# imaginateit/csm-train-pytorch

Measured on AMD Instinct MI355X. Metric: train tokens/sec (text+audio) CSM-1B bf16 seq2048, higher is better.
Workload: dtype bf16

## Files before the change

csm-train-pytorch_amd/csm/hip/__init__.py:

```python
import ctypes as C
import os

_HERE = os.path.dirname(os.path.abspath(__file__))
LIB_PATH = os.environ.get("CSM_HIP_LIB") or os.path.join(_HERE, "libcsm_hip.so")


class CsmHipError(RuntimeError):
    pass


if not os.path.exists(LIB_PATH):
    raise ImportError(
        f"{LIB_PATH} is missing: build it with `python __graft_entry__.py build` (or `make -C csm-train-pytorch_amd/csrc`). "
        "The CSM MI355X path has no fallback implementation."
    )

lib = C.CDLL(LIB_PATH)

_p, _i, _f, _ll = C.c_void_p, C.c_int, C.c_float, C.c_longlong

_SIGS = {
    "csm_abi_version": ([], _i),
    "csm_last_error": ([], C.c_char_p),
    "csm_device_check": ([_i], _i),
# ... 25 lines not shown
    "csm_set_attn_variant": ([_i], _i),
    "csm_attn_last_dkv_kernel": ([], _i),
    "csm_attn64_set_debug": ([_p], _i),
    "csm_set_decode_tuning": ([_i, _i], _i),
    "csm_attn_fwd": ([_p, _p, _p, _i, _i, _i, _i, _i, _p], _i),
    "csm_attn_bwd": ([_p, _p, _p, _p, _p, _p, _i, _i, _i, _i, _i, _p], _i),
    "csm_attn_bwd_rope": ([_p, _p, _p, _p, _p, _p, _p, _i, _i, _i, _i, _i, _p], _i),
    "csm_attn_fwd_seg": ([_p, _p, _p, _p, _i, _i, _i, _i, _i, _p], _i),
    "csm_attn_bwd_seg": ([_p, _p, _p, _p, _p, _p, _p, _p, _i, _i, _i, _i, _i, _p], _i),
    "csm_swiglu_fwd": ([_p, _p, _ll, _i, _p], _i),
    "csm_swiglu_bwd": ([_p, _p, _p, _ll, _i, _p], _i),
    "csm_embed_fwd": ([_p, _p, _p, _p, _p, _ll, _i, _i, _i, _p], _i),
    "csm_embed_bwd_sorted": ([_p, _p, _ll, _p, _p, _ll, _p, _p, _ll, _ll, _i, _p], _i),
    "csm_rows_add_bf16": ([_p, _p, _p, _ll, _i, _i, _p], _i),
    "csm_rows_take_bf16": ([_p, _p, _p, _ll, _i, _p], _i),
    "csm_decoder_input_fwd": ([_p, _p, _p, _p, _p, _ll, _i, _i, _i, _p], _i),
    "csm_ce_fwd_bwd": ([_p, _p, _p, _p, _ll, _i, _i, _i, _f, _p], _i),
    "csm_reduce_sum_f32": ([_p, _ll, _f, _p, _p], _i),
    "csm_sumsq_blocks": ([], _i),
    "csm_sumsq_bf16": ([_p, _ll, _p, _p], _i),
    "csm_clip_coef": ([_p, _i, _f, _p, _p], _i),
    "csm_adamw_step": ([_p, _p, _p, _p, _p, _ll, _f, _f, _f, _f, _f, _i, _p, _f, _i, _p], _i),
    "csm_adamw_step_split": ([_p, _p, _p, _p, _p, _ll, _f, _f, _f, _f, _f, _i, _p, _f, _i, _p], _i),
    "csm_set_adamw_blocks": ([_i], _i),
    "csm_gemv_bf16": ([_p, _p, _p, _p, _i, _i, _i, _i, _i, _i, _i, _p], _i),
    "csm_gemv_bf16_kext": ([_p, _p, _p, _p, _i, _i, _i, _i, _i, _i, _i, _p, _f, _i, _p, _i, _p, _p, _i, _i, _i, _p, _p], _i),
    "csm_lora_project_bf16": ([_p, _p, _p, _i, _i, _i, _i, _i, _i, _f, _p, _f, _p], _i),
    "csm_lora_project_rows_bf16": ([_p, _p, _p, _p, _p, _i, _i, _i, _i, _i, _i, _i, _p, _f, _p], _i),
    "csm_gemv_bf16_kext_rows": ([_p, _p, _p, _p, _i, _i, _i, _i, _i, _i, _i, _p, _f, _i, _p, _i, _p, _p, _p, _p, _i, _i, _i, _i, _p], _i),
    "csm_gemv_t_bf16": ([_p, _p, _p, _i, _i, _i, _i, _i, _i, _i, _p], _i),
    "csm_gemv_bf16_ex": ([_p, _p, _p, _p, _i, _i, _i, _i, _i, _i, _i, _p, _f, _i, _p, _i, _p], _i),
    "csm_quantize_rows_fp8": ([_p, _p, _p, _i, _i, _i, _i, _p], _i),
    "csm_gemv_fp8w": ([_p, _p, _p, _p, _p, _i, _i, _i, _i, _i, _i, _i, _p, _f, _i, _p, _i, _p], _i),
    "csm_attn_decode_rope": ([_p, _p, _p, _p, _p, _p, _i, _i, _i, _i, _i, _i, _p], _i),
    "csm_gemv_attn_bf16": ([_p, _p, _p, _p, _p, _p, _p, _p, _i, _i, _i, _i, _i, _i, _i, _i, _i, _p], _i),
    "csm_gemv_attn_at_bf16": ([_p, _p, _p, _i, _p, _p, _p, _p, _i, _i, _i, _i, _i, _i, _p], _i),
    "csm_attn_decode_rope_at": ([_p, _p, _p, _p, _i, _p, _i, _i, _i, _i, _i, _i, _p], _i),
    "csm_attn_append": ([_p, _p, _p, _p, _i, _i, _i, _i, _i, _i, _i, _f, _p], _i),
    "csm_attn_append_rows": ([_p, _p, _p, _p, _p, _p, _p, _i, _i, _i, _i, _i, _f, _p], _i),
    "csm_kv_append": ([_p, _p, _p, _p, _i, _i, _i, _i, _i, _i, _p], _i),
    "csm_kv_shift": ([_p, _p, _p, _i, _i, _i, _i, _i, _i, _i, _p], _i),
    "csm_attn_decode": ([_p, _p, _p, _p, _p, _i, _i, _i, _i, _i, _i, _p], _i),
    "csm_sample_topk": ([_p, _p, _p, _i, _i, _i, _i, _f, _p], _i),
    "csm_sample_topk_rows": ([_p, _p, _p, _i, _i, _i, _p, _p, _p], _i),
    "csm_sample_filtered_rows": ([_p, _p, _p, _i, _i, _i, _p, _p, _p, _p, _p], _i),
    "csm_rvq_encode": ([_p, _p, _p, _i, _i, _i, _i, _i, _p], _i),
# ... 60 lines not shown
```

csm-train-pytorch_amd/csm/hip/ops.py:

```python
import ctypes
import math
from typing import Optional

import torch

from . import CsmHipError, check, lib

BF16 = torch.bfloat16


def _stream() -> int:
    return torch.cuda.current_stream().cuda_stream


def _ptr(t: Optional[torch.Tensor]) -> Optional[int]:
    return None if t is None else t.data_ptr()


def _mat(t: torch.Tensor, dtype=BF16):
    assert t.is_cuda and t.dtype == dtype and t.dim() == 2 and t.stride(1) == 1, (t.dtype, t.shape, t.stride())
    return t.data_ptr(), t.shape[0], t.shape[1], t.stride(0)


def _pin(pin):
# ... 337 lines not shown
    R, ldl = logits_f32.shape[0], logits_f32.stride(0)
    assert logits_f32.dtype == torch.float32 and targets.dtype == torch.int64 and targets.is_contiguous()
    ldd = dlogits.stride(0) if dlogits is not None else 0
    check(lib.csm_ce_fwd_bwd(logits_f32.data_ptr(), targets.data_ptr(), loss_rows.data_ptr(), _ptr(dlogits), R, V, ldl, ldd,
                             float(grad_scale), _stream()), "csm_ce_fwd_bwd")


def reduce_sum(x_f32, out_f32, scale=1.0):
    check(lib.csm_reduce_sum_f32(x_f32.data_ptr(), x_f32.numel(), float(scale), out_f32.data_ptr(), _stream()), "csm_reduce_sum_f32")


def sumsq_blocks() -> int:
    return lib.csm_sumsq_blocks()


def sumsq_bf16(g, partials):
    check(lib.csm_sumsq_bf16(g.data_ptr(), g.numel(), partials.data_ptr(), _stream()), "csm_sumsq_bf16")


def clip_coef(partials, max_norm, norm_and_coef):
    check(lib.csm_clip_coef(partials.data_ptr(), partials.numel(), float(max_norm), norm_and_coef.data_ptr(), _stream()), "csm_clip_coef")


def adamw_step(master, m, v, param, grad, lr, beta1, beta2, eps, wd, step, norm_and_coef=None, grad_mul=1.0, zero_grad=False):
    n = master.numel()
    assert master.dtype == torch.float32 and param.dtype == BF16 and grad.dtype == BF16 and param.numel() == n == grad.numel()
    check(lib.csm_adamw_step(master.data_ptr(), m.data_ptr(), v.data_ptr(), param.data_ptr(), grad.data_ptr(), n, lr, beta1,
                             beta2, eps, wd, int(step), _ptr(norm_and_coef), float(grad_mul), int(zero_grad), _stream()), "csm_adamw_step")


def adamw_step_split(master_lo, m, v, param, grad, lr, beta1, beta2, eps, wd, step, norm_and_coef=None, grad_mul=1.0, zero_grad=False):
    n = master_lo.numel()
    assert master_lo.dtype == torch.int16 and param.dtype == BF16 and grad.dtype == BF16 and param.numel() == n == grad.numel()
    check(lib.csm_adamw_step_split(master_lo.data_ptr(), m.data_ptr(), v.data_ptr(), param.data_ptr(), grad.data_ptr(), n, lr, beta1,
                                   beta2, eps, wd, int(step), _ptr(norm_and_coef), float(grad_mul), int(zero_grad), _stream()),
          "csm_adamw_step_split")


def gemv(x, W, y, residual=None):
    B, K = x.shape
    N = W.shape[0]
    assert W.shape[1] == K and y.shape == (B, N) and x.stride(1) == 1 and W.stride(1) == 1 and y.stride(1) == 1
    check(lib.csm_gemv_bf16(x.data_ptr(), W.data_ptr(), y.data_ptr(), _ptr(residual), B, N, K, W.stride(0), x.stride(0),
                            y.stride(0), int(y.dtype == torch.float32), _stream()), "csm_gemv_bf16")
    return y


def gemv_ex(x, W, y, residual=None, norm_scale=None, eps=1e-5, swiglu=False, row_index=None, row_offset=0):
    B = y.shape[0]
    K = x.shape[1]
    N = W.shape[0]
    assert W.shape[1] == K and y.shape == (B, N // 2 if swiglu else N) and x.stride(1) == 1 and W.stride(1) == 1 and y.stride(1) == 1
    assert row_index is not None or x.shape[0] == B
    assert row_index is None or (row_index.dtype == torch.int32 and row_index.numel() == B and row_index.is_contiguous())
    check(lib.csm_gemv_bf16_ex(x.data_ptr(), W.data_ptr(), y.data_ptr(), _ptr(residual), B, N, K, W.stride(0), x.stride(0),
                               y.stride(0), int(y.dtype == torch.float32), _ptr(norm_scale), float(eps), int(swiglu),
                               _ptr(row_index), int(row_offset), _stream()), "csm_gemv_bf16_ex")
    return y

# ... 409 lines not shown
```

csm-train-pytorch_amd/csm/training/optim.py:

```python
import os
from typing import Dict, List, Optional

import torch

from ..hip import ops

F32 = torch.float32
SPLIT_MASTER = os.environ.get("CSM_ADAMW_SPLIT", "1") == "1"


def split_master(master: torch.Tensor, param_out: torch.Tensor) -> torch.Tensor:
    bits = master.contiguous().view(torch.int32)
    param_out.view(torch.int16).copy_(((bits + 0x8000) >> 16).to(torch.int16))
    return (bits & 0xFFFF).to(torch.int16)


def join_master(param: torch.Tensor, lo: torch.Tensor) -> torch.Tensor:
    hi = param.view(torch.int16).to(torch.int32) & 0xFFFF
    l = lo.to(torch.int32) & 0xFFFF
    return (((hi - (l >> 15)) << 16) | l).view(torch.float32)


def seed_master(model, offset: int, numel: int, param: torch.Tensor, from_fp32_source: bool = False) -> torch.Tensor:
    master = param.float()
    src = getattr(model, "_fp32_source", None) if from_fp32_source else None
    if src:
        views, base = model._views(model.arena), model.arena.storage_offset()
        for k, t in src.items():
            v = views.get(k)
            if v is None:
                continue
            so = v.storage_offset() - base
            end = _span_end(v, so)
            if so >= offset and end <= offset + numel:
                torch.as_strided(master, v.size(), v.stride(), so - offset).copy_(t.to(master.device))
            elif so < offset + numel and end > offset:
                a_, b_ = max(so, offset), min(end, offset + numel)
                scratch = torch.zeros(end - so, dtype=master.dtype, device=master.device)
                scratch[a_ - so:b_ - so] = master[a_ - offset:b_ - offset]
                torch.as_strided(scratch, v.size(), v.stride(), 0).copy_(t.to(master.device))
                master[a_ - offset:b_ - offset] = scratch[a_ - so:b_ - so]
    return master


def _span_end(v: torch.Tensor, so: int) -> int:
    return so + sum((sz - 1) * st for sz, st in zip(v.size(), v.stride())) + 1


class FusedAdamW:
    sharded = False

    def __init__(self, model, group_lrs: Dict[str, float], weight_decay: float = 0.01, betas=(0.9, 0.999),
                 eps: float = 1e-8, lora_lr: Optional[float] = None, lora_weight_decay: float = 0.0):
        self.model = model
        self.betas, self.eps = betas, eps
        self.param_groups: List[dict] = []
        self.state: Dict[str, Dict[str, torch.Tensor]] = {}
        self.step_count = 0
        self._coef: Optional[torch.Tensor] = None
        model.ensure_grads()
        for name, lr in group_lrs.items():
            if lr is None or not model.trainable.get(name, False):
                continue
            off, n = model.group_range(name)
            self.param_groups.append(dict(name=name, lr=float(lr), weight_decay=weight_decay, offset=off, numel=n,
                                          param=model.arena[off:off + n], grad=model.grad_arena[off:off + n]))
        if model.lora is not None and lora_lr is not None:
            lo = model.lora
            self.param_groups.append(dict(name="lora", lr=float(lora_lr), weight_decay=lora_weight_decay, offset=0,
                                          numel=lo.arena.numel(), param=lo.arena, grad=lo.grad_arena))
        for g in self.param_groups:
            master = self._seed_master(g, from_fp32_source=True)
            if SPLIT_MASTER:
                lo = split_master(master, g["param"])
                self.state[g["name"]] = dict(lo=lo, m=torch.zeros_like(master), v=torch.zeros_like(master))
                del master
            else:
                self.state[g["name"]] = dict(master=master, m=torch.zeros_like(master), v=torch.zeros_like(master))
        self._partials = torch.empty(max(1, len(self.param_groups)) * ops.sumsq_blocks(), dtype=F32, device=model.device)
        self._norm_coef = torch.ones(2, dtype=F32, device=model.device)
        import weakref
        if not hasattr(model, "_optimizers"):
            model._optimizers = []
        model._optimizers.append(weakref.ref(self))

    def _seed_master(self, g, from_fp32_source: bool = False) -> torch.Tensor:
        return seed_master(self.model, g["offset"], g["numel"], g["param"], from_fp32_source and g["name"] != "lora")

    def named_master(self):
        m = self.model
        views, base = m._views(m.arena), m.arena.storage_offset()
        for g in self.param_groups:
            if g["name"] == "lora":
                continue
            master = self.master(g["name"])
            for k, v in views.items():
                so = v.storage_offset() - base
                if g["offset"] <= so < g["offset"] + g["numel"]:
                    yield k, torch.as_strided(master, v.size(), v.stride(), so - g["offset"])

    def _group(self, name):
        return next(g for g in self.param_groups if g["name"] == name)

    def master(self, name: str) -> torch.Tensor:
        st = self.state[name]
        return st["master"] if "master" in st else join_master(self._group(name)["param"], st["lo"])

    def set_master(self, name: str, master: torch.Tensor):
        st, g = self.state[name], self._group(name)
        if "master" in st:
# ... 24 lines not shown
        nb = ops.sumsq_blocks()
        for i, g in enumerate(self.param_groups):
            ops.sumsq_bf16(g["grad"], self._partials[i * nb:(i + 1) * nb])
        ops.clip_coef(self._partials[:len(self.param_groups) * nb], max_norm, self._norm_coef)
        self._coef = self._norm_coef
        return self._norm_coef[0]

    def step(self, zero_grad=False, skip: Optional[torch.Tensor] = None):
        self._settle()
        self.step_count += 1
        self.model._fp32_source = None
        if skip is not None:
            coef = self._coef[1] if self._coef is not None else torch.ones((), dtype=F32, device=skip.device)
            self._norm_coef[1] = torch.where(skip.reshape(()) != 0, torch.full_like(coef, -1.0), coef)
            self._coef = self._norm_coef
        b1, b2 = self.betas
        gs = self.model.grad_state
        for g in self.param_groups:
            st = self.state[g["name"]]
            name = g["name"]
            zero = bool(zero_grad) if zero_grad != "lazy" else (name == "embeddings" or name not in gs)
            if "lo" in st:
                ops.adamw_step_split(st["lo"], st["m"], st["v"], g["param"], g["grad"], g["lr"], b1, b2, self.eps,
                                     g["weight_decay"], self.step_count, self._coef, zero_grad=zero)
            else:
                ops.adamw_step(st["master"], st["m"], st["v"], g["param"], g["grad"], g["lr"], b1, b2, self.eps,
                               g["weight_decay"], self.step_count, self._coef, zero_grad=zero)
            if name in gs:
                if zero:
                    gs[name] = "zero"
                elif zero_grad == "lazy" and gs[name] == "live":
                    gs[name] = "stale"
        self._coef = None

    def uncount_step(self):
        self.step_count = max(0, self.step_count - 1)

    def params_rewritten(self, base: bool = True, lora: bool = True, from_fp32_source: bool = False):
        for g in self.param_groups:
            if lora if g["name"] == "lora" else base:
                self.set_master(g["name"], self._seed_master(g, from_fp32_source))

    def state_dict(self):
        return {"step": self.step_count,
                "groups": [{k: g[k] for k in ("name", "lr", "weight_decay", "offset", "numel")} for g in self.param_groups],
                "state": {n: {"master": self.master(n).cpu(), "m": st["m"].cpu(), "v": st["v"].cpu()} for n, st in self.state.items()}}

    def load_state_dict(self, sd):
        saved_by_name = {g["name"]: g for g in sd["groups"]}
        mine = [g["name"] for g in self.param_groups]
        if sorted(saved_by_name) != sorted(mine) or sorted(sd["state"]) != sorted(mine):
            raise ValueError(f"optimizer state was saved for parameter groups {sorted(saved_by_name)} but this optimizer has "
                             f"{sorted(mine)} (different freeze flags / LoRA setting?)")
        for g in self.param_groups:
            saved = saved_by_name[g["name"]]
            if (saved["offset"], saved["numel"]) != (g["offset"], g["numel"]):
                raise ValueError(f"optimizer group {g['name']!r}: saved range {saved['offset']}+{saved['numel']} != {g['offset']}+{g['numel']}")
        self.step_count = sd["step"]
        for n, st in sd["state"].items():
            for k, v in st.items():
                if k == "master":
                    self.set_master(n, v)
                else:
                    self.state[n][k].copy_(v)
        for g in self.param_groups:
            saved = saved_by_name[g["name"]]
            g["lr"], g["weight_decay"] = saved["lr"], saved["weight_decay"]
```

csm-train-pytorch_amd/csrc/ops.hip:

```cpp
#include "common.h"
#include <math.h>

namespace {

template <int NC>
__global__ __launch_bounds__(256) void rmsnorm_fwd_kernel(const bf16_t* __restrict__ x, const bf16_t* __restrict__ w,
                                                          bf16_t* __restrict__ y, float* __restrict__ rstd, int M, int D,
                                                          float eps) {
    const int lane = threadIdx.x & 63;
    const int wpb = blockDim.x >> 6;
    const int nchunk = D >> 3;
    for (long long row = (long long)blockIdx.x * wpb + (threadIdx.x >> 6); row < M; row += (long long)gridDim.x * wpb) {
        U4 v[NC];
        float ss = 0.f;
#pragma unroll
        for (int i = 0; i < NC; ++i) {
            const int c = lane + 64 * i;
            v[i] = (U4){0u, 0u, 0u, 0u};
            if (c < nchunk) v[i] = *reinterpret_cast<const U4*>(x + (size_t)row * D + c * 8);
            float f[8];
            unpack8(v[i], f);
#pragma unroll
            for (int j = 0; j < 8; ++j) ss += f[j] * f[j];
        }
// ... 502 lines not shown
        unpack8(*reinterpret_cast<const U4*>(g + i * 8), f);
#pragma unroll
        for (int j = 0; j < 8; ++j) acc += f[j] * f[j];
    }
    if (blockIdx.x == 0)
        for (long long i = (nvec << 3) + threadIdx.x; i < n; i += blockDim.x) { const float f = bf2f(g[i]); acc += f * f; }
    acc = block_sum(acc, red);
    if (threadIdx.x == 0) partials[blockIdx.x] = acc;
}

__global__ __launch_bounds__(1024) void clip_coef_kernel(const float* __restrict__ partials, int n, float max_norm,
                                                         float* __restrict__ out) {
    __shared__ float red[16];
    float acc = 0.f;
    for (int i = threadIdx.x; i < n; i += blockDim.x) acc += partials[i];
    acc = block_sum(acc, red);
    if (threadIdx.x == 0) {
        const float norm = sqrtf(acc);
        out[0] = norm;
        out[1] = (max_norm > 0.f) ? fminf(1.f, max_norm / (norm + 1e-6f)) : 1.f;
    }
}

__device__ __forceinline__ void adam_update(float& p, float& m, float& v, float g, float lr, float beta1, float beta2, float eps,
                                            float wd, float bc1, float bc2_sqrt) {
#pragma clang fp contract(off)
    p = p * (1.f - lr * wd);
    m = beta1 * m + (1.f - beta1) * g;
    v = beta2 * v + ((1.f - beta2) * g) * g;
    const float denom = sqrtf(v) / bc2_sqrt + eps;
    p = p - (lr / bc1) * (m / denom);
}

__device__ __forceinline__ void adamw_skipped(bf16_t* __restrict__ grad, long long nvec, int zero_grad) {
    if (!zero_grad) return;
    for (long long i = (long long)blockIdx.x * blockDim.x + threadIdx.x; i < nvec; i += (long long)gridDim.x * blockDim.x)
        *reinterpret_cast<U4*>(grad + i * 8) = (U4){0u, 0u, 0u, 0u};
}

__global__ __launch_bounds__(256) void adamw_kernel(float* __restrict__ master, float* __restrict__ m, float* __restrict__ v,
                                                    bf16_t* __restrict__ param, bf16_t* __restrict__ grad, long long n,
                                                    float lr, float beta1, float beta2, float eps, float wd, float bc1,
                                                    float bc2_sqrt, const float* __restrict__ coef_ptr, float gmul,
                                                    int zero_grad) {
    const float coef = (coef_ptr ? coef_ptr[1] : 1.f) * gmul;
    const long long nvec = n >> 3;
    if (coef_ptr && coef_ptr[1] < 0.f) { adamw_skipped(grad, nvec, zero_grad); return; }
    for (long long i = (long long)blockIdx.x * blockDim.x + threadIdx.x; i < nvec; i += (long long)gridDim.x * blockDim.x) {
        float g[8];
        unpack8(*reinterpret_cast<const U4*>(grad + i * 8), g);
        float4 p0 = *reinterpret_cast<const float4*>(master + i * 8), p1 = *reinterpret_cast<const float4*>(master + i * 8 + 4);
        float4 m0 = *reinterpret_cast<const float4*>(m + i * 8), m1 = *reinterpret_cast<const float4*>(m + i * 8 + 4);
        float4 v0 = *reinterpret_cast<const float4*>(v + i * 8), v1 = *reinterpret_cast<const float4*>(v + i * 8 + 4);
        float p[8] = {p0.x, p0.y, p0.z, p0.w, p1.x, p1.y, p1.z, p1.w};
        float mm[8] = {m0.x, m0.y, m0.z, m0.w, m1.x, m1.y, m1.z, m1.w};
        float vv[8] = {v0.x, v0.y, v0.z, v0.w, v1.x, v1.y, v1.z, v1.w};
#pragma unroll
        for (int j = 0; j < 8; ++j) {
            adam_update(p[j], mm[j], vv[j], g[j] * coef, lr, beta1, beta2, eps, wd, bc1, bc2_sqrt);
        }
        *reinterpret_cast<float4*>(master + i * 8) = make_float4(p[0], p[1], p[2], p[3]);
        *reinterpret_cast<float4*>(master + i * 8 + 4) = make_float4(p[4], p[5], p[6], p[7]);
        *reinterpret_cast<float4*>(m + i * 8) = make_float4(mm[0], mm[1], mm[2], mm[3]);
        *reinterpret_cast<float4*>(m + i * 8 + 4) = make_float4(mm[4], mm[5], mm[6], mm[7]);
        *reinterpret_cast<float4*>(v + i * 8) = make_float4(vv[0], vv[1], vv[2], vv[3]);
        *reinterpret_cast<float4*>(v + i * 8 + 4) = make_float4(vv[4], vv[5], vv[6], vv[7]);
        *reinterpret_cast<U4*>(param + i * 8) = pack8(p);
        if (zero_grad) *reinterpret_cast<U4*>(grad + i * 8) = (U4){0u, 0u, 0u, 0u};
    }
}

__global__ __launch_bounds__(256) void adamw_split_kernel(uint16_t* __restrict__ lo, float* __restrict__ m, float* __restrict__ v,
                                                          bf16_t* __restrict__ param, bf16_t* __restrict__ grad, long long n,
                                                          float lr, float beta1, float beta2, float eps, float wd, float bc1,
                                                          float bc2_sqrt, const float* __restrict__ coef_ptr, float gmul,
                                                          int zero_grad) {
    const float coef = (coef_ptr ? coef_ptr[1] : 1.f) * gmul;
    const long long nvec = n >> 3;
    if (coef_ptr && coef_ptr[1] < 0.f) { adamw_skipped(grad, nvec, zero_grad); return; }
    for (long long i = (long long)blockIdx.x * blockDim.x + threadIdx.x; i < nvec; i += (long long)gridDim.x * blockDim.x) {
        float g[8];
        unpack8(*reinterpret_cast<const U4*>(grad + i * 8), g);
        const U4 hw = *reinterpret_cast<const U4*>(param + i * 8), lw = *reinterpret_cast<const U4*>(lo + i * 8);
        float4 m0 = *reinterpret_cast<const float4*>(m + i * 8), m1 = *reinterpret_cast<const float4*>(m + i * 8 + 4);
        float4 v0 = *reinterpret_cast<const float4*>(v + i * 8), v1 = *reinterpret_cast<const float4*>(v + i * 8 + 4);
        const uint32_t hww[4] = {hw.x, hw.y, hw.z, hw.w}, lww[4] = {lw.x, lw.y, lw.z, lw.w};
        float p[8];
#pragma unroll
        for (int j = 0; j < 8; ++j) {
            const uint32_t h16 = (hww[j >> 1] >> ((j & 1) * 16)) & 0xffffu, l16 = (lww[j >> 1] >> ((j & 1) * 16)) & 0xffffu;
            p[j] = __uint_as_float(((h16 - (l16 >> 15)) << 16) | l16);
        }
        float mm[8] = {m0.x, m0.y, m0.z, m0.w, m1.x, m1.y, m1.z, m1.w};
        float vv[8] = {v0.x, v0.y, v0.z, v0.w, v1.x, v1.y, v1.z, v1.w};
        uint32_t ho[4] = {0u, 0u, 0u, 0u}, lout[4] = {0u, 0u, 0u, 0u};
#pragma unroll
        for (int j = 0; j < 8; ++j) {
            adam_update(p[j], mm[j], vv[j], g[j] * coef, lr, beta1, beta2, eps, wd, bc1, bc2_sqrt);
            const uint32_t bits = __float_as_uint(p[j]);
            ho[j >> 1] |= (((bits + 0x8000u) >> 16) & 0xffffu) << ((j & 1) * 16);
            lout[j >> 1] |= (bits & 0xffffu) << ((j & 1) * 16);
        }
        *reinterpret_cast<float4*>(m + i * 8) = make_float4(mm[0], mm[1], mm[2], mm[3]);
        *reinterpret_cast<float4*>(m + i * 8 + 4) = make_float4(mm[4], mm[5], mm[6], mm[7]);
        *reinterpret_cast<float4*>(v + i * 8) = make_float4(vv[0], vv[1], vv[2], vv[3]);
        *reinterpret_cast<float4*>(v + i * 8 + 4) = make_float4(vv[4], vv[5], vv[6], vv[7]);
        *reinterpret_cast<U4*>(param + i * 8) = (U4){ho[0], ho[1], ho[2], ho[3]};
        *reinterpret_cast<U4*>(lo + i * 8) = (U4){lout[0], lout[1], lout[2], lout[3]};
        if (zero_grad) *reinterpret_cast<U4*>(grad + i * 8) = (U4){0u, 0u, 0u, 0u};
    }
}

inline int grid_for(long long work_items, int block, int cap = 256 * 8) {
    long long b = (work_items + block - 1) / block;
    if (b < 1) b = 1;
    return (int)(b > cap ? cap : b);
}

}

extern "C" int csm_rmsnorm_fwd(const void* x, const void* scale, void* y, float* rstd, int M, int D, float eps,
                               hipStream_t stream) {
    CSM_REQUIRE(x && scale && y, "csm_rmsnorm_fwd: null pointer");
    CSM_REQUIRE(M > 0 && D > 0 && (D & 7) == 0 && D <= 4096, "csm_rmsnorm_fwd: D=%d must be a multiple of 8 and <= 4096", D);
    const int grid = grid_for(M, 4, 4096);
    const int nc = (D + 511) / 512;
#define L(NC) hipLaunchKernelGGL((rmsnorm_fwd_kernel<NC>), dim3(grid), dim3(256), 0, stream, (const bf16_t*)x, (const bf16_t*)scale, (bf16_t*)y, rstd, M, D, eps)
    if (nc <= 1) L(1); else if (nc <= 2) L(2); else if (nc <= 4) L(4); else L(8);
#undef L
    CSM_CHECK_LAUNCH("csm_rmsnorm_fwd");
    return 0;
}
// ... 201 lines not shown
                              const float* norm_and_coef, float grad_mul, int zero_grad, hipStream_t stream) {
    CSM_REQUIRE(master && m && v && param && grad && n > 0 && step > 0, "csm_adamw_step: bad arguments");
    CSM_REQUIRE((n & 7) == 0, "csm_adamw_step: n must be a multiple of 8 (pad the arena)");
    const float bc1 = 1.f - powf(beta1, (float)step);
    const float bc2s = sqrtf(1.f - powf(beta2, (float)step));
    hipLaunchKernelGGL(adamw_kernel, dim3(grid_for(n >> 3, 256, g_adamw_blocks)), dim3(256), 0, stream, master, m, v, (bf16_t*)param,
                       (bf16_t*)grad, n, lr, beta1, beta2, eps, weight_decay, bc1, bc2s, norm_and_coef, grad_mul, zero_grad);
    CSM_CHECK_LAUNCH("csm_adamw_step");
    return 0;
}

extern "C" int csm_adamw_step_split(void* master_lo, float* m, float* v, void* param, void* grad, long long n, float lr, float beta1,
                                    float beta2, float eps, float weight_decay, int step, const float* norm_and_coef, float grad_mul,
                                    int zero_grad, hipStream_t stream) {
    CSM_REQUIRE(master_lo && m && v && param && grad && n > 0 && step >= 1, "csm_adamw_step_split: bad arguments");
    CSM_REQUIRE((n & 7) == 0, "csm_adamw_step_split: n must be a multiple of 8 (pad the arena)");
    const float bc1 = 1.f - powf(beta1, (float)step);
    const float bc2s = sqrtf(1.f - powf(beta2, (float)step));
    hipLaunchKernelGGL(adamw_split_kernel, dim3(grid_for(n >> 3, 256, g_adamw_blocks)), dim3(256), 0, stream, (uint16_t*)master_lo, m, v,
                       (bf16_t*)param, (bf16_t*)grad, n, lr, beta1, beta2, eps, weight_decay, bc1, bc2s, norm_and_coef, grad_mul, zero_grad);
    CSM_CHECK_LAUNCH("csm_adamw_step_split");
    return 0;
}
```

include/csm_hip.h:

```cpp
#ifndef CSM_HIP_H
#define CSM_HIP_H
#include <stdint.h>

#ifdef __cplusplus
extern "C" {
#endif

typedef struct ihipStream_t* csm_stream_t;

int csm_abi_version(void);
const char* csm_last_error(void);
int csm_device_check(int device);

int csm_gemm_bf16(const void* A, const void* B, void* C, const void* R, int M, int N, int K, int lda, int ldb, int ldc,
                  int ldr, int transA, int transB, int out_f32, float alpha, int batch, long long strideA,
                  long long strideB, long long strideC, long long strideR, csm_stream_t stream);

int csm_gemm_bf16_ex(const void* A, const void* B, void* C, const void* R, int M, int N, int K, int lda, int ldb, int ldc,
                     int ldr, int transA, int transB, int out_f32, float alpha, int batch, long long strideA,
                     long long strideB, long long strideC, long long strideR, int epilogue, const void* aux_in,
                     void* aux_out, int ld_aux, csm_stream_t stream);
int csm_gemm_bf16_rope(const void* A, const void* W, void* C, int M, int N, int K, int lda, int ldw, int ldc,
                       const float* rope_table, int rows_per_seq, int n_rope_cols, int head_dim, csm_stream_t stream);
int csm_gemm_bf16_kext(const void* A, const void* B, void* C, const void* R, int M, int N, int K, int lda, int ldb, int ldc, int ldr,
// ... 60 lines not shown

int csm_embed_bwd_sorted(const long long* sorted_rows, const long long* src_index, long long n_occ, const void* dh,
                         const void* dseq, long long M, void* g_text, void* g_audio, long long text_rows, long long n_rows,
                         int D, csm_stream_t stream);
int csm_rows_add_bf16(void* dst, const int* rows, const void* src, long long N, int src_stride_rows, int D, csm_stream_t stream);
int csm_rows_take_bf16(void* table, const int* rows, void* out, long long N, int D, csm_stream_t stream);

int csm_decoder_input_fwd(const void* hidden, const int* rows, const long long* codes, const void* audio_emb, void* out,
                          long long N, int K, int D, int audio_vocab, csm_stream_t stream);

int csm_ce_fwd_bwd(const float* logits, const long long* targets, float* loss_rows, void* dlogits, long long R, int V,
                   int ldl, int ldd, float grad_scale, csm_stream_t stream);
int csm_reduce_sum_f32(const float* x, long long n, float scale, float* out, csm_stream_t stream);

int csm_sumsq_blocks(void);
int csm_sumsq_bf16(const void* g, long long n, float* partials , csm_stream_t stream);
int csm_clip_coef(const float* partials, int n_partials, float max_norm, float* norm_and_coef , csm_stream_t stream);
int csm_adamw_step(float* master, float* m, float* v, void* param, void* grad, long long n, float lr, float beta1,
                   float beta2, float eps, float weight_decay, int step, const float* norm_and_coef ,
                   float grad_mul, int zero_grad , csm_stream_t stream);
int csm_adamw_step_split(void* master_lo, float* m, float* v, void* param, void* grad, long long n, float lr, float beta1,
                         float beta2, float eps, float weight_decay, int step, const float* norm_and_coef, float grad_mul,
                         int zero_grad, csm_stream_t stream);

int csm_set_adamw_blocks(int blocks);

int csm_sample_topk(const float* logits, const float* q, int* out, int rows, int V, int ldl, int topk, float temperature,
                    csm_stream_t stream);
int csm_sample_topk_rows(const float* logits, const float* q, int* out, int rows, int V, int ldl, const int* topk,
                         const float* temperature, csm_stream_t stream);
int csm_sample_filtered_rows(const float* logits, const float* q, int* out, int rows, int V, int ldl, const int* topk,
                             const float* temperature, const float* top_p, const float* min_p, csm_stream_t stream);

int csm_set_decode_tuning(int key, int value);
int csm_gemv_bf16(const void* x, const void* W, void* y, const void* residual, int B, int N, int K, int ldw, int ldx, int ldy,
                  int out_f32, csm_stream_t stream);
int csm_gemv_bf16_ex(const void* x, const void* W, void* y, const void* residual, int B, int N, int K, int ldw, int ldx, int ldy,
                     int out_f32, const void* norm_scale, float eps, int swiglu, const int* row_index, int row_offset,
                     csm_stream_t stream);
int csm_quantize_rows_fp8(const void* W, void* W8, void* scale, int N, int K, int ldw, int ldw8, csm_stream_t stream);
int csm_gemv_fp8w(const void* x, const void* W8, const void* scale, void* y, const void* residual, int B, int N, int K, int ldw8,
                  int ldx, int ldy, int out_f32, const void* norm_scale, float eps, int swiglu, const int* row_index, int row_offset,
                  csm_stream_t stream);
int csm_lora_project_bf16(const void* x, const void* At, void* t, int B, int K, int kx, int ldx, int lda, int ldt, float scale,
                          const void* norm_scale, float eps, csm_stream_t stream);
int csm_gemv_bf16_kext(const void* x, const void* W, void* y, const void* residual, int B, int N, int K, int ldw, int ldx, int ldy,
// ... 85 lines not shown
```

Measured before the change: 129,100.

## Skip moment reads and writes for never-touched embedding blocks in AdamW

Adds per-2048-element liveness flags for the embeddings group so the AdamW kernel can skip reading and writing m/v in blocks whose moments are still zero and whose gradient is zero. Such blocks only get weight decay applied, and that shortcut is taken only when a zero-gradient update is bit-exactly a no-op. Blocks are marked live once they receive any gradient, and the flags are recomputed after a checkpoint load. This cuts optimizer memory traffic for large, sparsely hit embedding tables, at the cost of a block-wide OR-reduction and an extra flag buffer.

```diff
diff --git a/csm-train-pytorch_amd/csm/hip/__init__.py b/csm-train-pytorch_amd/csm/hip/__init__.py
--- a/csm-train-pytorch_amd/csm/hip/__init__.py
+++ b/csm-train-pytorch_amd/csm/hip/__init__.py
@@ -71,6 +71,8 @@
     "csm_clip_coef": ([_p, _i, _f, _p, _p], _i),
     "csm_adamw_step": ([_p, _p, _p, _p, _p, _ll, _f, _f, _f, _f, _f, _i, _p, _f, _i, _p], _i),
     "csm_adamw_step_split": ([_p, _p, _p, _p, _p, _ll, _f, _f, _f, _f, _f, _i, _p, _f, _i, _p], _i),
+    "csm_adamw_step_live": ([_p, _p, _p, _p, _p, _ll, _f, _f, _f, _f, _f, _i, _p, _f, _i, _p, _p], _i),
+    "csm_adamw_step_split_live": ([_p, _p, _p, _p, _p, _ll, _f, _f, _f, _f, _f, _i, _p, _f, _i, _p, _p], _i),
     "csm_set_adamw_blocks": ([_i], _i),
     "csm_gemv_bf16": ([_p, _p, _p, _p, _i, _i, _i, _i, _i, _i, _i, _p], _i),
     "csm_gemv_bf16_kext": ([_p, _p, _p, _p, _i, _i, _i, _i, _i, _i, _i, _p, _f, _i, _p, _i, _p, _p, _i, _i, _i, _p, _p], _i),
diff --git a/csm-train-pytorch_amd/csm/hip/ops.py b/csm-train-pytorch_amd/csm/hip/ops.py
--- a/csm-train-pytorch_amd/csm/hip/ops.py
+++ b/csm-train-pytorch_amd/csm/hip/ops.py
@@ -383,19 +383,36 @@
     check(lib.csm_clip_coef(partials.data_ptr(), partials.numel(), float(max_norm), norm_and_coef.data_ptr(), _stream()), "csm_clip_coef")
 
 
-def adamw_step(master, m, v, param, grad, lr, beta1, beta2, eps, wd, step, norm_and_coef=None, grad_mul=1.0, zero_grad=False):
+ADAMW_BLOCK = 2048
+
+
+def _live_ptr(block_live, n):
+    assert block_live.dtype == torch.uint8 and block_live.is_contiguous() and block_live.numel() == -(-n // ADAMW_BLOCK)
+    return block_live.data_ptr()
+
+
+def adamw_step(master, m, v, param, grad, lr, beta1, beta2, eps, wd, step, norm_and_coef=None, grad_mul=1.0, zero_grad=False, *,
+               block_live=None):
     n = master.numel()
     assert master.dtype == torch.float32 and param.dtype == BF16 and grad.dtype == BF16 and param.numel() == n == grad.numel()
-    check(lib.csm_adamw_step(master.data_ptr(), m.data_ptr(), v.data_ptr(), param.data_ptr(), grad.data_ptr(), n, lr, beta1,
-                             beta2, eps, wd, int(step), _ptr(norm_and_coef), float(grad_mul), int(zero_grad), _stream()), "csm_adamw_step")
-
-
-def adamw_step_split(master_lo, m, v, param, grad, lr, beta1, beta2, eps, wd, step, norm_and_coef=None, grad_mul=1.0, zero_grad=False):
+    args = (master.data_ptr(), m.data_ptr(), v.data_ptr(), param.data_ptr(), grad.data_ptr(), n, lr, beta1, beta2, eps, wd, int(step),
+            _ptr(norm_and_coef), float(grad_mul), int(zero_grad))
+    if block_live is None:
+        check(lib.csm_adamw_step(*args, _stream()), "csm_adamw_step")
+    else:
+        check(lib.csm_adamw_step_live(*args, _live_ptr(block_live, n), _stream()), "csm_adamw_step_live")
+
+
+def adamw_step_split(master_lo, m, v, param, grad, lr, beta1, beta2, eps, wd, step, norm_and_coef=None, grad_mul=1.0, zero_grad=False, *,
+                     block_live=None):
     n = master_lo.numel()
     assert master_lo.dtype == torch.int16 and param.dtype == BF16 and grad.dtype == BF16 and param.numel() == n == grad.numel()
-    check(lib.csm_adamw_step_split(master_lo.data_ptr(), m.data_ptr(), v.data_ptr(), param.data_ptr(), grad.data_ptr(), n, lr, beta1,
-                                   beta2, eps, wd, int(step), _ptr(norm_and_coef), float(grad_mul), int(zero_grad), _stream()),
-          "csm_adamw_step_split")
+    args = (master_lo.data_ptr(), m.data_ptr(), v.data_ptr(), param.data_ptr(), grad.data_ptr(), n, lr, beta1, beta2, eps, wd, int(step),
+            _ptr(norm_and_coef), float(grad_mul), int(zero_grad))
+    if block_live is None:
+        check(lib.csm_adamw_step_split(*args, _stream()), "csm_adamw_step_split")
+    else:
+        check(lib.csm_adamw_step_split_live(*args, _live_ptr(block_live, n), _stream()), "csm_adamw_step_split_live")
 
 
 def gemv(x, W, y, residual=None):
diff --git a/csm-train-pytorch_amd/csm/training/optim.py b/csm-train-pytorch_amd/csm/training/optim.py
--- a/csm-train-pytorch_amd/csm/training/optim.py
+++ b/csm-train-pytorch_amd/csm/training/optim.py
@@ -7,6 +7,7 @@
 
 F32 = torch.float32
 SPLIT_MASTER = os.environ.get("CSM_ADAMW_SPLIT", "1") == "1"
+FLAGGED_GROUPS = ("embeddings",)
 
 
 def split_master(master: torch.Tensor, param_out: torch.Tensor) -> torch.Tensor:
@@ -47,8 +48,18 @@
     return so + sum((sz - 1) * st for sz, st in zip(v.size(), v.stride())) + 1
 
 
+def live_blocks(m: torch.Tensor, v: torch.Tensor) -> torch.Tensor:
+    bits, B = m.view(torch.int32) | v.view(torch.int32), ops.ADAMW_BLOCK
+    full = bits.numel() // B * B
+    live = [bits[:full].view(-1, B).any(dim=1)]
+    if full < bits.numel():
+        live.append(bits[full:].any().reshape(1))
+    return torch.cat(live).to(torch.uint8)
+
+
 class FusedAdamW:
     sharded = False
+    dead_blocks = True
 
     def __init__(self, model, group_lrs: Dict[str, float], weight_decay: float = 0.01, betas=(0.9, 0.999),
                  eps: float = 1e-8, lora_lr: Optional[float] = None, lora_weight_decay: float = 0.0):
@@ -58,6 +69,7 @@
         self.state: Dict[str, Dict[str, torch.Tensor]] = {}
         self.step_count = 0
         self._coef: Optional[torch.Tensor] = None
+        self.dead_blocks = os.environ.get("CSM_ADAMW_DEAD_BLOCKS", "1") == "1"
         model.ensure_grads()
         for name, lr in group_lrs.items():
             if lr is None or not model.trainable.get(name, False):
@@ -77,6 +89,8 @@
                 del master
             else:
                 self.state[g["name"]] = dict(master=master, m=torch.zeros_like(master), v=torch.zeros_like(master))
+            if self.dead_blocks and g["name"] in FLAGGED_GROUPS:
+                self.state[g["name"]]["live"] = torch.zeros(-(-g["numel"] // ops.ADAMW_BLOCK), dtype=torch.uint8, device=g["param"].device)
         self._partials = torch.empty(max(1, len(self.param_groups)) * ops.sumsq_blocks(), dtype=F32, device=model.device)
         self._norm_coef = torch.ones(2, dtype=F32, device=model.device)
         import weakref
@@ -86,6 +100,12 @@
 
     def _seed_master(self, g, from_fp32_source: bool = False) -> torch.Tensor:
         return seed_master(self.model, g["offset"], g["numel"], g["param"], from_fp32_source and g["name"] != "lora")
+
+    def moments_rewritten(self):
+        for name in FLAGGED_GROUPS:
+            if self.dead_blocks and name in self.state:
+                st = self.state[name]
+                st["live"] = live_blocks(st["m"], st["v"])
 
     def named_master(self):
         m = self.model
@@ -156,10 +176,10 @@
             zero = bool(zero_grad) if zero_grad != "lazy" else (name == "embeddings" or name not in gs)
             if "lo" in st:
                 ops.adamw_step_split(st["lo"], st["m"], st["v"], g["param"], g["grad"], g["lr"], b1, b2, self.eps,
-                                     g["weight_decay"], self.step_count, self._coef, zero_grad=zero)
+                                     g["weight_decay"], self.step_count, self._coef, zero_grad=zero, block_live=st.get("live"))
             else:
                 ops.adamw_step(st["master"], st["m"], st["v"], g["param"], g["grad"], g["lr"], b1, b2, self.eps,
-                               g["weight_decay"], self.step_count, self._coef, zero_grad=zero)
+                               g["weight_decay"], self.step_count, self._coef, zero_grad=zero, block_live=st.get("live"))
             if name in gs:
                 if zero:
                     gs[name] = "zero"
@@ -197,6 +217,7 @@
                     self.set_master(n, v)
                 else:
                     self.state[n][k].copy_(v)
+        self.moments_rewritten()
         for g in self.param_groups:
             saved = saved_by_name[g["name"]]
             g["lr"], g["weight_decay"] = saved["lr"], saved["weight_decay"]
diff --git a/csm-train-pytorch_amd/csrc/ops.hip b/csm-train-pytorch_amd/csrc/ops.hip
--- a/csm-train-pytorch_amd/csrc/ops.hip
+++ b/csm-train-pytorch_amd/csrc/ops.hip
@@ -548,20 +548,60 @@
     }
 }
 
+__device__ __forceinline__ float adam_decay(float p, float lr, float wd) {
+#pragma clang fp contract(off)
+    return p * (1.f - lr * wd);
+}
+
+__device__ __forceinline__ float adam_moments(float& m, float& v, float g, float lr, float beta1, float beta2, float eps, float bc1,
+                                              float bc2_sqrt) {
+#pragma clang fp contract(off)
+    m = beta1 * m + (1.f - beta1) * g;
+    v = beta2 * v + ((1.f - beta2) * g) * g;
+    const float denom = sqrtf(v) / bc2_sqrt + eps;
+    return (lr / bc1) * (m / denom);
+}
+
 __device__ __forceinline__ void adam_update(float& p, float& m, float& v, float g, float lr, float beta1, float beta2, float eps,
                                             float wd, float bc1, float bc2_sqrt) {
 #pragma clang fp contract(off)
-    p = p * (1.f - lr * wd);
-    m = beta1 * m + (1.f - beta1) * g;
-    v = beta2 * v + ((1.f - beta2) * g) * g;
-    const float denom = sqrtf(v) / bc2_sqrt + eps;
-    p = p - (lr / bc1) * (m / denom);
+    p = adam_decay(p, lr, wd);
+    p = p - adam_moments(m, v, g, lr, beta1, beta2, eps, bc1, bc2_sqrt);
 }
 
 __device__ __forceinline__ void adamw_skipped(bf16_t* __restrict__ grad, long long nvec, int zero_grad) {
     if (!zero_grad) return;
     for (long long i = (long long)blockIdx.x * blockDim.x + threadIdx.x; i < nvec; i += (long long)gridDim.x * blockDim.x)
         *reinterpret_cast<U4*>(grad + i * 8) = (U4){0u, 0u, 0u, 0u};
+}
+
+struct AdamArgs {
+    float lr, beta1, beta2, eps, wd, bc1, bc2_sqrt, coef;
+    int zero_grad;
+};
+
+__device__ __forceinline__ void adamw_vec(float* __restrict__ master, float* __restrict__ m, float* __restrict__ v,
+                                          bf16_t* __restrict__ param, bf16_t* __restrict__ grad, long long i, const AdamArgs& a) {
+    float g[8];
+    unpack8(*reinterpret_cast<const U4*>(grad + i * 8), g);
+    float4 p0 = *reinterpret_cast<const float4*>(master + i * 8), p1 = *reinterpret_cast<const float4*>(master + i * 8 + 4);
+    float4 m0 = *reinterpret_cast<const float4*>(m + i * 8), m1 = *reinterpret_cast<const float4*>(m + i * 8 + 4);
+    float4 v0 = *reinterpret_cast<const float4*>(v + i * 8), v1 = *reinterpret_cast<const float4*>(v + i * 8 + 4);
+    float p[8] = {p0.x, p0.y, p0.z, p0.w, p1.x, p1.y, p1.z, p1.w};
+    float mm[8] = {m0.x, m0.y, m0.z, m0.w, m1.x, m1.y, m1.z, m1.w};
+    float vv[8] = {v0.x, v0.y, v0.z, v0.w, v1.x, v1.y, v1.z, v1.w};
+#pragma unroll
+    for (int j = 0; j < 8; ++j) {
+        adam_update(p[j], mm[j], vv[j], g[j] * a.coef, a.lr, a.beta1, a.beta2, a.eps, a.wd, a.bc1, a.bc2_sqrt);
+    }
+    *reinterpret_cast<float4*>(master + i * 8) = make_float4(p[0], p[1], p[2], p[3]);
+    *reinterpret_cast<float4*>(master + i * 8 + 4) = make_float4(p[4], p[5], p[6], p[7]);
+    *reinterpret_cast<float4*>(m + i * 8) = make_float4(mm[0], mm[1], mm[2], mm[3]);
+    *reinterpret_cast<float4*>(m + i * 8 + 4) = make_float4(mm[4], mm[5], mm[6], mm[7]);
+    *reinterpret_cast<float4*>(v + i * 8) = make_float4(vv[0], vv[1], vv[2], vv[3]);
+    *reinterpret_cast<float4*>(v + i * 8 + 4) = make_float4(vv[4], vv[5], vv[6], vv[7]);
+    *reinterpret_cast<U4*>(param + i * 8) = pack8(p);
+    if (a.zero_grad) *reinterpret_cast<U4*>(grad + i * 8) = (U4){0u, 0u, 0u, 0u};
 }
 
 __global__ __launch_bounds__(256) void adamw_kernel(float* __restrict__ master, float* __restrict__ m, float* __restrict__ v,
@@ -572,28 +612,43 @@
     const float coef = (coef_ptr ? coef_ptr[1] : 1.f) * gmul;
     const long long nvec = n >> 3;
     if (coef_ptr && coef_ptr[1] < 0.f) { adamw_skipped(grad, nvec, zero_grad); return; }
+    const AdamArgs a = {lr, beta1, beta2, eps, wd, bc1, bc2_sqrt, coef, zero_grad};
     for (long long i = (long long)blockIdx.x * blockDim.x + threadIdx.x; i < nvec; i += (long long)gridDim.x * blockDim.x) {
-        float g[8];
-        unpack8(*reinterpret_cast<const U4*>(grad + i * 8), g);
-        float4 p0 = *reinterpret_cast<const float4*>(master + i * 8), p1 = *reinterpret_cast<const float4*>(master + i * 8 + 4);
-        float4 m0 = *reinterpret_cast<const float4*>(m + i * 8), m1 = *reinterpret_cast<const float4*>(m + i * 8 + 4);
-        float4 v0 = *reinterpret_cast<const float4*>(v + i * 8), v1 = *reinterpret_cast<const float4*>(v + i * 8 + 4);
-        float p[8] = {p0.x, p0.y, p0.z, p0.w, p1.x, p1.y, p1.z, p1.w};
-        float mm[8] = {m0.x, m0.y, m0.z, m0.w, m1.x, m1.y, m1.z, m1.w};
-        float vv[8] = {v0.x, v0.y, v0.z, v0.w, v1.x, v1.y, v1.z, v1.w};
-#pragma unroll
-        for (int j = 0; j < 8; ++j) {
-            adam_update(p[j], mm[j], vv[j], g[j] * coef, lr, beta1, beta2, eps, wd, bc1, bc2_sqrt);
-        }
-        *reinterpret_cast<float4*>(master + i * 8) = make_float4(p[0], p[1], p[2], p[3]);
-        *reinterpret_cast<float4*>(master + i * 8 + 4) = make_float4(p[4], p[5], p[6], p[7]);
-        *reinterpret_cast<float4*>(m + i * 8) = make_float4(mm[0], mm[1], mm[2], mm[3]);
-        *reinterpret_cast<float4*>(m + i * 8 + 4) = make_float4(mm[4], mm[5], mm[6], mm[7]);
-        *reinterpret_cast<float4*>(v + i * 8) = make_float4(vv[0], vv[1], vv[2], vv[3]);
-        *reinterpret_cast<float4*>(v + i * 8 + 4) = make_float4(vv[4], vv[5], vv[6], vv[7]);
-        *reinterpret_cast<U4*>(param + i * 8) = pack8(p);
-        if (zero_grad) *reinterpret_cast<U4*>(grad + i * 8) = (U4){0u, 0u, 0u, 0u};
-    }
+        adamw_vec(master, m, v, param, grad, i, a);
+    }
+}
+
+__device__ __forceinline__ void adamw_split_vec(uint16_t* __restrict__ lo, float* __restrict__ m, float* __restrict__ v,
+                                                bf16_t* __restrict__ param, bf16_t* __restrict__ grad, long long i, const AdamArgs& a) {
+    float g[8];
+    unpack8(*reinterpret_cast<const U4*>(grad + i * 8), g);
+    const U4 hw = *reinterpret_cast<const U4*>(param + i * 8), lw = *reinterpret_cast<const U4*>(lo + i * 8);
+    float4 m0 = *reinterpret_cast<const float4*>(m + i * 8), m1 = *reinterpret_cast<const float4*>(m + i * 8 + 4);
+    float4 v0 = *reinterpret_cast<const float4*>(v + i * 8), v1 = *reinterpret_cast<const float4*>(v + i * 8 + 4);
+    const uint32_t hww[4] = {hw.x, hw.y, hw.z, hw.w}, lww[4] = {lw.x, lw.y, lw.z, lw.w};
+    float p[8];
+#pragma unroll
+    for (int j = 0; j < 8; ++j) {
+        const uint32_t h16 = (hww[j >> 1] >> ((j & 1) * 16)) & 0xffffu, l16 = (lww[j >> 1] >> ((j & 1) * 16)) & 0xffffu;
+        p[j] = __uint_as_float(((h16 - (l16 >> 15)) << 16) | l16);
+    }
+    float mm[8] = {m0.x, m0.y, m0.z, m0.w, m1.x, m1.y, m1.z, m1.w};
+    float vv[8] = {v0.x, v0.y, v0.z, v0.w, v1.x, v1.y, v1.z, v1.w};
+    uint32_t ho[4] = {0u, 0u, 0u, 0u}, lout[4] = {0u, 0u, 0u, 0u};
+#pragma unroll
+    for (int j = 0; j < 8; ++j) {
+        adam_update(p[j], mm[j], vv[j], g[j] * a.coef, a.lr, a.beta1, a.beta2, a.eps, a.wd, a.bc1, a.bc2_sqrt);
+        const uint32_t bits = __float_as_uint(p[j]);
+        ho[j >> 1] |= (((bits + 0x8000u) >> 16) & 0xffffu) << ((j & 1) * 16);
+        lout[j >> 1] |= (bits & 0xffffu) << ((j & 1) * 16);
+    }
+    *reinterpret_cast<float4*>(m + i * 8) = make_float4(mm[0], mm[1], mm[2], mm[3]);
+    *reinterpret_cast<float4*>(m + i * 8 + 4) = make_float4(mm[4], mm[5], mm[6], mm[7]);
+    *reinterpret_cast<float4*>(v + i * 8) = make_float4(vv[0], vv[1], vv[2], vv[3]);
+    *reinterpret_cast<float4*>(v + i * 8 + 4) = make_float4(vv[4], vv[5], vv[6], vv[7]);
+    *reinterpret_cast<U4*>(param + i * 8) = (U4){ho[0], ho[1], ho[2], ho[3]};
+    *reinterpret_cast<U4*>(lo + i * 8) = (U4){lout[0], lout[1], lout[2], lout[3]};
+    if (a.zero_grad) *reinterpret_cast<U4*>(grad + i * 8) = (U4){0u, 0u, 0u, 0u};
 }
 
 __global__ __launch_bounds__(256) void adamw_split_kernel(uint16_t* __restrict__ lo, float* __restrict__ m, float* __restrict__ v,
@@ -604,36 +659,95 @@
     const float coef = (coef_ptr ? coef_ptr[1] : 1.f) * gmul;
     const long long nvec = n >> 3;
     if (coef_ptr && coef_ptr[1] < 0.f) { adamw_skipped(grad, nvec, zero_grad); return; }
+    const AdamArgs a = {lr, beta1, beta2, eps, wd, bc1, bc2_sqrt, coef, zero_grad};
     for (long long i = (long long)blockIdx.x * blockDim.x + threadIdx.x; i < nvec; i += (long long)gridDim.x * blockDim.x) {
-        float g[8];
-        unpack8(*reinterpret_cast<const U4*>(grad + i * 8), g);
-        const U4 hw = *reinterpret_cast<const U4*>(param + i * 8), lw = *reinterpret_cast<const U4*>(lo + i * 8);
-        float4 m0 = *reinterpret_cast<const float4*>(m + i * 8), m1 = *reinterpret_cast<const float4*>(m + i * 8 + 4);
-        float4 v0 = *reinterpret_cast<const float4*>(v + i * 8), v1 = *reinterpret_cast<const float4*>(v + i * 8 + 4);
-        const uint32_t hww[4] = {hw.x, hw.y, hw.z, hw.w}, lww[4] = {lw.x, lw.y, lw.z, lw.w};
-        float p[8];
-#pragma unroll
-        for (int j = 0; j < 8; ++j) {
-            const uint32_t h16 = (hww[j >> 1] >> ((j & 1) * 16)) & 0xffffu, l16 = (lww[j >> 1] >> ((j & 1) * 16)) & 0xffffu;
-            p[j] = __uint_as_float(((h16 - (l16 >> 15)) << 16) | l16);
-        }
-        float mm[8] = {m0.x, m0.y, m0.z, m0.w, m1.x, m1.y, m1.z, m1.w};
-        float vv[8] = {v0.x, v0.y, v0.z, v0.w, v1.x, v1.y, v1.z, v1.w};
-        uint32_t ho[4] = {0u, 0u, 0u, 0u}, lout[4] = {0u, 0u, 0u, 0u};
-#pragma unroll
-        for (int j = 0; j < 8; ++j) {
-            adam_update(p[j], mm[j], vv[j], g[j] * coef, lr, beta1, beta2, eps, wd, bc1, bc2_sqrt);
-            const uint32_t bits = __float_as_uint(p[j]);
-            ho[j >> 1] |= (((bits + 0x8000u) >> 16) & 0xffffu) << ((j & 1) * 16);
-            lout[j >> 1] |= (bits & 0xffffu) << ((j & 1) * 16);
-        }
-        *reinterpret_cast<float4*>(m + i * 8) = make_float4(mm[0], mm[1], mm[2], mm[3]);
-        *reinterpret_cast<float4*>(m + i * 8 + 4) = make_float4(mm[4], mm[5], mm[6], mm[7]);
-        *reinterpret_cast<float4*>(v + i * 8) = make_float4(vv[0], vv[1], vv[2], vv[3]);
-        *reinterpret_cast<float4*>(v + i * 8 + 4) = make_float4(vv[4], vv[5], vv[6], vv[7]);
-        *reinterpret_cast<U4*>(param + i * 8) = (U4){ho[0], ho[1], ho[2], ho[3]};
-        *reinterpret_cast<U4*>(lo + i * 8) = (U4){lout[0], lout[1], lout[2], lout[3]};
-        if (zero_grad) *reinterpret_cast<U4*>(grad + i * 8) = (U4){0u, 0u, 0u, 0u};
+        adamw_split_vec(lo, m, v, param, grad, i, a);
+    }
+}
+
+__device__ __forceinline__ bool adam_dead_exact(const AdamArgs& a) {
+    float m = 0.f, v = 0.f;
+    const float t = adam_moments(m, v, 0.f * a.coef, a.lr, a.beta1, a.beta2, a.eps, a.bc1, a.bc2_sqrt);
+    return (__float_as_uint(m) | __float_as_uint(v) | __float_as_uint(t)) == 0u;
+}
+
+__global__ __launch_bounds__(256) void adamw_live_kernel(float* __restrict__ master, float* __restrict__ m, float* __restrict__ v,
+                                                         bf16_t* __restrict__ param, bf16_t* __restrict__ grad, long long n,
+                                                         float lr, float beta1, float beta2, float eps, float wd, float bc1,
+                                                         float bc2_sqrt, const float* __restrict__ coef_ptr, float gmul,
+                                                         int zero_grad, uint8_t* block_live) {
+    const AdamArgs a = {lr, beta1, beta2, eps, wd, bc1, bc2_sqrt, (coef_ptr ? coef_ptr[1] : 1.f) * gmul, zero_grad};
+    const long long nvec = n >> 3, nblk = (nvec + 255) >> 8;
+    if (coef_ptr && coef_ptr[1] < 0.f) { adamw_skipped(grad, nvec, zero_grad); return; }
+    const bool dead_exact = adam_dead_exact(a);
+    for (long long b = blockIdx.x; b < nblk; b += gridDim.x) {
+        const long long i = b * 256 + threadIdx.x;
+        const bool in = i < nvec;
+        const bool live = block_live[b] != 0;
+        U4 gw = {0u, 0u, 0u, 0u};
+        float4 p0 = {0.f, 0.f, 0.f, 0.f}, p1 = p0;
+        if (in) {
+            gw = *reinterpret_cast<const U4*>(grad + i * 8);
+            p0 = *reinterpret_cast<const float4*>(master + i * 8), p1 = *reinterpret_cast<const float4*>(master + i * 8 + 4);
+        }
+        if (!live) {
+            const bool any = __syncthreads_or((gw.x | gw.y | gw.z | gw.w) != 0u) != 0;
+            if (!any && dead_exact) {
+                if (in) {
+                    float p[8] = {p0.x, p0.y, p0.z, p0.w, p1.x, p1.y, p1.z, p1.w};
+#pragma unroll
+                    for (int j = 0; j < 8; ++j) p[j] = adam_decay(p[j], lr, wd);
+                    *reinterpret_cast<float4*>(master + i * 8) = make_float4(p[0], p[1], p[2], p[3]);
+                    *reinterpret_cast<float4*>(master + i * 8 + 4) = make_float4(p[4], p[5], p[6], p[7]);
+                    *reinterpret_cast<U4*>(param + i * 8) = pack8(p);
+                }
+                continue;
+            }
+            if (threadIdx.x == 0) block_live[b] = 1;
+        }
+        if (in) adamw_vec(master, m, v, param, grad, i, a);
+    }
+}
+
+__global__ __launch_bounds__(256) void adamw_split_live_kernel(uint16_t* __restrict__ lo, float* __restrict__ m, float* __restrict__ v,
+                                                               bf16_t* __restrict__ param, bf16_t* __restrict__ grad, long long n,
+                                                               float lr, float beta1, float beta2, float eps, float wd, float bc1,
+                                                               float bc2_sqrt, const float* __restrict__ coef_ptr, float gmul,
+                                                               int zero_grad, uint8_t* block_live) {
+    const AdamArgs a = {lr, beta1, beta2, eps, wd, bc1, bc2_sqrt, (coef_ptr ? coef_ptr[1] : 1.f) * gmul, zero_grad};
+    const long long nvec = n >> 3, nblk = (nvec + 255) >> 8;
+    if (coef_ptr && coef_ptr[1] < 0.f) { adamw_skipped(grad, nvec, zero_grad); return; }
+    const bool dead_exact = adam_dead_exact(a);
+    for (long long b = blockIdx.x; b < nblk; b += gridDim.x) {
+        const long long i = b * 256 + threadIdx.x;
+        const bool in = i < nvec;
+        const bool live = block_live[b] != 0;
+        U4 gw = {0u, 0u, 0u, 0u}, hw = gw, lw = gw;
+        if (in) {
+            gw = *reinterpret_cast<const U4*>(grad + i * 8);
+            hw = *reinterpret_cast<const U4*>(param + i * 8), lw = *reinterpret_cast<const U4*>(lo + i * 8);
+        }
+        if (!live) {
+            const bool any = __syncthreads_or((gw.x | gw.y | gw.z | gw.w) != 0u) != 0;
+            if (!any && dead_exact) {
+                if (in) {
+                    const uint32_t hww[4] = {hw.x, hw.y, hw.z, hw.w}, lww[4] = {lw.x, lw.y, lw.z, lw.w};
+                    uint32_t ho[4] = {0u, 0u, 0u, 0u}, lout[4] = {0u, 0u, 0u, 0u};
+#pragma unroll
+                    for (int j = 0; j < 8; ++j) {
+                        const uint32_t h16 = (hww[j >> 1] >> ((j & 1) * 16)) & 0xffffu, l16 = (lww[j >> 1] >> ((j & 1) * 16)) & 0xffffu;
+                        const uint32_t bits = __float_as_uint(adam_decay(__uint_as_float(((h16 - (l16 >> 15)) << 16) | l16), lr, wd));
+                        ho[j >> 1] |= (((bits + 0x8000u) >> 16) & 0xffffu) << ((j & 1) * 16);
+                        lout[j >> 1] |= (bits & 0xffffu) << ((j & 1) * 16);
+                    }
+                    *reinterpret_cast<U4*>(param + i * 8) = (U4){ho[0], ho[1], ho[2], ho[3]};
+                    *reinterpret_cast<U4*>(lo + i * 8) = (U4){lout[0], lout[1], lout[2], lout[3]};
+                }
+                continue;
+            }
+            if (threadIdx.x == 0) block_live[b] = 1;
+        }
+        if (in) adamw_split_vec(lo, m, v, param, grad, i, a);
     }
 }
 
@@ -881,3 +995,32 @@
     CSM_CHECK_LAUNCH("csm_adamw_step_split");
     return 0;
 }
+
+extern "C" int csm_adamw_step_live(float* master, float* m, float* v, void* param, void* grad, long long n, float lr,
+                                   float beta1, float beta2, float eps, float weight_decay, int step,
+                                   const float* norm_and_coef, float grad_mul, int zero_grad, void* block_live, hipStream_t stream) {
+    CSM_REQUIRE(master && m && v && param && grad && block_live && n > 0 && step > 0, "csm_adamw_step_live: bad arguments");
+    CSM_REQUIRE((n & 7) == 0, "csm_adamw_step_live: n must be a multiple of 8 (pad the arena)");
+    const float bc1 = 1.f - powf(beta1, (float)step);
+    const float bc2s = sqrtf(1.f - powf(beta2, (float)step));
+    hipLaunchKernelGGL(adamw_live_kernel, dim3(grid_for(n >> 3, 256, g_adamw_blocks)), dim3(256), 0, stream, master, m, v, (bf16_t*)param,
+                       (bf16_t*)grad, n, lr, beta1, beta2, eps, weight_decay, bc1, bc2s, norm_and_coef, grad_mul, zero_grad,
+                       (uint8_t*)block_live);
+    CSM_CHECK_LAUNCH("csm_adamw_step_live");
+    return 0;
+}
+
+extern "C" int csm_adamw_step_split_live(void* master_lo, float* m, float* v, void* param, void* grad, long long n, float lr,
+                                         float beta1, float beta2, float eps, float weight_decay, int step,
+                                         const float* norm_and_coef, float grad_mul, int zero_grad, void* block_live,
+                                         hipStream_t stream) {
+    CSM_REQUIRE(master_lo && m && v && param && grad && block_live && n > 0 && step >= 1, "csm_adamw_step_split_live: bad arguments");
+    CSM_REQUIRE((n & 7) == 0, "csm_adamw_step_split_live: n must be a multiple of 8 (pad the arena)");
+    const float bc1 = 1.f - powf(beta1, (float)step);
+    const float bc2s = sqrtf(1.f - powf(beta2, (float)step));
+    hipLaunchKernelGGL(adamw_split_live_kernel, dim3(grid_for(n >> 3, 256, g_adamw_blocks)), dim3(256), 0, stream, (uint16_t*)master_lo,
+                       m, v, (bf16_t*)param, (bf16_t*)grad, n, lr, beta1, beta2, eps, weight_decay, bc1, bc2s, norm_and_coef, grad_mul,
+                       zero_grad, (uint8_t*)block_live);
+    CSM_CHECK_LAUNCH("csm_adamw_step_split_live");
+    return 0;
+}
diff --git a/include/csm_hip.h b/include/csm_hip.h
--- a/include/csm_hip.h
+++ b/include/csm_hip.h
@@ -106,6 +106,12 @@
 int csm_adamw_step_split(void* master_lo, float* m, float* v, void* param, void* grad, long long n, float lr, float beta1,
                          float beta2, float eps, float weight_decay, int step, const float* norm_and_coef, float grad_mul,
                          int zero_grad, csm_stream_t stream);
+int csm_adamw_step_live(float* master, float* m, float* v, void* param, void* grad, long long n, float lr, float beta1,
+                        float beta2, float eps, float weight_decay, int step, const float* norm_and_coef, float grad_mul,
+                        int zero_grad, void* block_live, csm_stream_t stream);
+int csm_adamw_step_split_live(void* master_lo, float* m, float* v, void* param, void* grad, long long n, float lr, float beta1,
+                              float beta2, float eps, float weight_decay, int step, const float* norm_and_coef, float grad_mul,
+                              int zero_grad, void* block_live, csm_stream_t stream);
 
 int csm_set_adamw_blocks(int blocks);
 
```

Result: faster. 130,600, median of 6 (+1.2%).
